# rishihahs/pupperv3-mjx

Measured on AMD Instinct MI355X. Metric: env-steps/sec at N_envs=4096/GPU, 1/2/4/8 MI355X; qpos rel-err vs mj_step, higher is better.
Workload: dtype f32

## Files before the change

### pupperv3-mjx_amd/csrc/pp3_device.h

```cpp
#pragma once
#include <hip/hip_runtime.h>
#include <stdint.h>

#include "pupper_hip.h"

namespace pp3 {

constexpr int NB = PP3_NBODY;
constexpr int NJ = PP3_NJNT;
constexpr int NV = PP3_NV;
constexpr int NQ = PP3_NQ;
constexpr int NU = PP3_NU;
constexpr int WAVE = 64;
constexpr int NLMAX = 12;
constexpr int NFR = 12;
constexpr int MAX_ROBOT_GEOM = 16;
constexpr int NMPAIR_MAX = 128;
constexpr int NMPAIR = 117;
constexpr int PAIR_REC = 24;

enum { PK_PLANE_SPHERE = 0, PK_SPHERE_SPHERE = 1, PK_SPHERE_BOX = 2 };
struct alignas(16) PairRec {
  int32_t kind, s1, s2;
  float r1, r2, margin;
  float p1[3], p2[3];
  float R[9];
  float half[3];
};
static_assert(sizeof(PairRec) == PAIR_REC * 4, "PairRec layout");
struct alignas(16) TerrainRec {
  float p[3];
  float R[9];
  float half[3];
  float pad;
};
static_assert(sizeof(TerrainRec) == 64, "TerrainRec layout");
struct alignas(16) PairCon {
  int32_t sup;
  uint32_t dm[2];
  float mu;
  float tran;
  float margin, b, k;
  float solimp[5];
  float knee, body;
  float pad;
};
static_assert(sizeof(PairCon) == 64, "PairCon layout");
static_assert(offsetof(PairCon, knee) == 52, "PairCon: knee/body in the 4th 16-byte word group");

template <int N>
struct alignas(16) LaneRec {
  float f[4 * N];
};
template <int N>
struct alignas(16) LaneTab {
  float g[N][32][4];
};
struct alignas(16) PairTab {
  float g[PAIR_REC / 4][PP3_MAX_PAIR][4];
};
enum {
  LL_LIM_ON = 0, LL_RANGE, LL_MARGIN, LL_INVW, LL_B, LL_K, LL_SOLIMP,
  LL_FR_R = 11, LL_FR_B, LL_ACT_DOF, LL_ACT_QADR, LL_ACT_FLAGS, LL_CRANGE,
  LL_GEAR = 18, LL_GAIN, LL_BIAS,
  LL_FRANGE = 23,
  LL_WORDS = 25
};
enum { ACTF_CTRLLIMITED = 1, ACTF_FORCELIMITED = 2, ACTF_AFFINE = 4 };
enum { LC_IQUAT = 0, LC_PT_BODY = 4, LC_PT_POS = 5, LC_WORDS = 8 };
enum { LM_IJ = 0, LM_ARM = 4, LM_DAMP = 8, LM_FLOSS = 9, LM_WORDS = 10 };
enum { LE_POSE = 0, LE_JLO, LE_JHI, LE_ABD, LE_LEG, LE_POSE16, LE_WORDS = 6 };
enum { LS_TYPE = 0, LS_ADR, LS_CUT, LS_BODY, LS_SPOS, LS_SQUAT = 7, LS_NCH = 11, LS_CH = 12, LS_MAXCH = 4,
       LS_WORDS = LS_CH + 4 * LS_MAXCH };

constexpr float MINVAL = 1e-15f;
constexpr float MINIMP = 0.0001f;
constexpr float MAXIMP = 0.9999f;

struct DevModel {
  LaneTab<(LL_WORDS + 3) / 4> lane_lim;
  LaneTab<(LC_WORDS + 3) / 4> lane_com;
  LaneTab<(LM_WORDS + 3) / 4> lane_m;
  float h;
  float gravity[3];
  float impratio;
  float gtol_scale;
  int32_t ls_iterations;
  int32_t iterations;
  float body_pos[NB][3];
  float body_quat[NB][4];
  float body_iquat[NB][4];
  float body_ipos[NB][3];
  float body_mass[NB];
// ... 283 lines not shown
```

### pupperv3-mjx_amd/csrc/pp3_env.hip

```cpp
#include <hip/hip_runtime.h>

#include <float.h>
#include <math.h>
#include <stddef.h>
#include <stdio.h>
#include <stdlib.h>
#include <string.h>

#include <string>
#include <algorithm>
#include <vector>

#include "pp3_device.h"
#include "pp3_diag.h"
#include "pp3_mlp.h"

namespace pp3 {

constexpr int HW = 32;
typedef __attribute__((address_space(4))) const DevModel GModel;
typedef __attribute__((address_space(4))) const float GFloat;
constexpr int HMAX = 16;
constexpr int OBS_MOVE = (PP3_OBS_DIM * (HMAX - 1) + HW - 1) / HW;
constexpr int NROBOT_GEOM = 8;
// ... 53 lines not shown
  float con_G[NC][5];
  float Jc[NC][3][NV];
  int lim_dof[NLMAX];
  float lim_sgn[NLMAX];
  float efc_D[NEFC], efc_R[NEFC], efc_aref[NEFC], efc_force[NEFC];
  Scratch<NC> x;
};

#define SYNC() asm volatile("" ::: "memory")
typedef float v4f __attribute__((ext_vector_type(4)));
#define PIN(...) asm volatile("" : __VA_ARGS__)
template <int N, int STRIDE>
__device__ __forceinline__ LaneRec<N> fetch_groups(const float* p) {
  v4f v[N];
#pragma unroll
  for (int k = 0; k < N; k++) v[k] = *reinterpret_cast<const v4f*>(p + k * STRIDE);
  if constexpr (N == 1) PIN("+v"(v[0]));
  else if constexpr (N == 2) PIN("+v"(v[0]), "+v"(v[1]));
  else if constexpr (N == 3) PIN("+v"(v[0]), "+v"(v[1]), "+v"(v[2]));
  else if constexpr (N == 4) PIN("+v"(v[0]), "+v"(v[1]), "+v"(v[2]), "+v"(v[3]));
  else if constexpr (N == 7) PIN("+v"(v[0]), "+v"(v[1]), "+v"(v[2]), "+v"(v[3]), "+v"(v[4]), "+v"(v[5]), "+v"(v[6]));
  else static_assert(N == 1, "fetch_rec: add a PIN arity");
  LaneRec<N> r;
#pragma unroll
  for (int k = 0; k < N; k++)
#pragma unroll
    for (int c = 0; c < 4; c++) r.f[4 * k + c] = v[k][c];
  return r;
}
template <int N>
__device__ __forceinline__ LaneRec<N> fetch_rec(const LaneRec<N>& src) {
  return fetch_groups<N, 4>(src.f);
}
template <int N>
__device__ __forceinline__ LaneRec<N> fetch_rec(const LaneTab<N>& t, int l) {
  return fetch_groups<N, 4 * 32>(t.g[0][l]);
}
__device__ __forceinline__ int as_i(float f) { return __float_as_int(f); }

__device__ __forceinline__ float frcp(float x) { return __builtin_amdgcn_rcpf(x); }
__device__ __forceinline__ float dpp_shr4(float v) {
  return __int_as_float(__builtin_amdgcn_update_dpp(0, __float_as_int(v), 0x114, 0xF, 0xF, true));
}

constexpr int HEAVY_WEIGHT = 5;

__device__ __forceinline__ float hb(float v, int k, int h) {
  const float a = rlane(v, k), b = rlane(v, k + HW);
  return h ? b : a;
}
__device__ __forceinline__ uint32_t hbu(uint32_t v, int k, int h) {
  const uint32_t a = (uint32_t)__builtin_amdgcn_readlane((int)v, k);
  const uint32_t b = (uint32_t)__builtin_amdgcn_readlane((int)v, k + HW);
  return h ? b : a;
}
__device__ __forceinline__ Key hkey(Key k, int l, int h) { return Key{hbu(k.a, l, h), hbu(k.b, l, h)}; }
__device__ __forceinline__ float hsum(float v, int) {
  v += dpp_f<0xB1, 0xF>(v, 0.0f);
  v += dpp_f<0x4E, 0xF>(v, 0.0f);
  v += dpp_f<0x141, 0xF>(v, 0.0f);
  v += dpp_f<0x140, 0xF>(v, 0.0f);
  const auto r = __builtin_amdgcn_permlane16_swap(__float_as_uint(v), __float_as_uint(v), false, false);
  return __uint_as_float(r[0]) + __uint_as_float(r[1]);
}
__device__ __forceinline__ float hsum_lane16(float v) {
  v += dpp_f<0xB1, 0xF>(v, 0.0f);
  v += dpp_f<0x4E, 0xF>(v, 0.0f);
  v += dpp_f<0x141, 0xF>(v, 0.0f);
  v += dpp_f<0x140, 0xF>(v, 0.0f);
// ... 250 lines not shown
    float t[10];
#pragma unroll
    for (int k = 0; k < 10; k++) t[k] = hsum_lane16(ci[k]);
    if (l == 16)
#pragma unroll
      for (int k = 0; k < 10; k++) s.crb_base[k] = t[k];
  }
  if (geom || foot) {
    float* dst = geom ? s.gxpos[l] : s.foot_xpos[l - 16];
    for (int k = 0; k < 3; k++) dst[k] = gpos[k];
  }
}

__device__ __forceinline__ void make_frame(float f[9], const float nin[3]) {
  float a[3] = {nin[0], nin[1], nin[2]};
  float n = sqrtf(dot3(a, a));
  if (n < MINVAL) { a[0] = 1; a[1] = 0; a[2] = 0; } else { const float in = 1.0f / n; a[0] *= in; a[1] *= in; a[2] *= in; }
  float y[3] = {0, 0, 0};
  if (a[1] < 0.5f && a[1] > -0.5f) y[1] = 1; else y[2] = 1;
  float ad = dot3(a, y);
  for (int k = 0; k < 3; k++) y[k] -= a[k] * ad;
  float yn = sqrtf(dot3(y, y));
  if (yn < MINVAL) { y[0] = 1; y[1] = 0; y[2] = 0; } else { const float in = 1.0f / yn; y[0] *= in; y[1] *= in; y[2] *= in; }
  float z[3];
  cross3(z, a, y);
  for (int k = 0; k < 3; k++) { f[k] = a[k]; f[3 + k] = y[k]; f[6 + k] = z[k]; }
}

struct PairLoad {
  v4f v[7];
};
__device__ __forceinline__ PairLoad load_pair(const DevModel& m, int p) {
  PairLoad r;
#pragma unroll
  for (int k = 0; k < 6; k++) r.v[k] = *reinterpret_cast<const v4f*>(m.pair_rec.g[k][p]);
  r.v[6] = *reinterpret_cast<const v4f*>(&m.pair_con[p]);
  return r;
}
struct TerrainRef {
  uint64_t terrain;
  int nbox;
};
template <int NC, int NWV = 1>
__device__ __forceinline__ bool narrow(const Shared<NC>& s, const TerrainRef& tr, PairLoad pl, float& dist, float pos[3],
                                       float nrm[3], v4f& pc0) {
  PairRec rec;
  {
    PIN("+v"(pl.v[0]), "+v"(pl.v[1]), "+v"(pl.v[2]), "+v"(pl.v[3]), "+v"(pl.v[4]), "+v"(pl.v[5]), "+v"(pl.v[6]));
    __builtin_memcpy(&rec, pl.v, sizeof(rec));
    pc0 = pl.v[6];
  }
  const float margin = rec.margin;
  float p1[3], p2[3];
  {
    const int i1 = rec.s1 >= 0 ? rec.s1 : 0, i2 = rec.s2 >= 0 ? rec.s2 : 0;
    float l1[3], l2[3];
#pragma unroll
    for (int k = 0; k < 3; k++) { l1[k] = s.gxpos[i1][k]; l2[k] = s.gxpos[i2][k]; }
    asm volatile("" : "+v"(l1[0]), "+v"(l1[1]), "+v"(l1[2]), "+v"(l2[0]), "+v"(l2[1]), "+v"(l2[2]));
#pragma unroll
    for (int k = 0; k < 3; k++) {
      p1[k] = rec.s1 >= 0 ? l1[k] : rec.p1[k];
      p2[k] = rec.s2 >= 0 ? l2[k] : rec.p2[k];
    }
  }
  if (rec.kind == PK_PLANE_SPHERE) {
    const float nz[3] = {rec.R[2], rec.R[5], rec.R[8]};
    const float v[3] = {p2[0] - p1[0], p2[1] - p1[1], p2[2] - p1[2]};
    const float r = rec.r2;
// ... 367 lines not shown
  for (int k = 0; k < NV - 1; ++k) {
    const float yk = hb(x, k, h);
    x = (l > k) ? x - a[k] * yk : x;
  }
  x = x * dinv;
  SYNC();
  float col[NV];
#pragma unroll
  for (int k = 1; k < NV; ++k) col[k] = s.x.L[k][li];
#pragma unroll
  for (int k = NV - 1; k > 0; --k) {
    const float xk = hb(x, k, h);
    x = (l < k) ? x - col[k] * xk : x;
  }
  return x;
}

__host__ __device__ constexpr int pnat(int p) { return p < 12 ? p + 6 : p - 12; }
__host__ __device__ constexpr int npos(int d) { return d < 6 ? d + 12 : d - 6; }

__device__ __forceinline__ float dpp_shl1(float v) { return dpp_f<0x101, 0xF>(v, 0.0f); }
__device__ __forceinline__ float dpp_shl2(float v) { return dpp_f<0x102, 0xF>(v, 0.0f); }

__device__ __forceinline__ float ldl_arrow_solve(float (&a)[NV], float b, int l, float* col ) {
  l = opaque_lane(l);
  const int slot = l < NV ? l : NV;
  const int lp = l < NV ? l : NV - 1;
  const int pg = lp < 12 ? lp / 3 : 0, pst = lp < 12 ? lp - 3 * pg : 3;
  float mydiag = 1.0f;
#pragma unroll
  for (int st = 0; st < 3; st++) {
#pragma unroll
    for (int g = 0; g < 4; g++) col[20 * g + slot] = a[3 * g + st];
    if (l < 12 && l - 3 * (l / 3) == st) col[20 * (l / 3) + 19] = b;
    SYNC();
    {
      const float pv = col[20 * pg + slot];
      mydiag = (pst == st) ? pv : mydiag;
    }
#pragma unroll
    for (int g = 0; g < 4; g++) {
      const int k = 3 * g + st;
      const float* c = col + 20 * g;
      float r[20];
#pragma unroll
      for (int qq = 0; qq < 2; qq++) {
        const int q = ((3 * g) & ~3) + 4 * qq;
        if (q < 12 && q <= 3 * g + 2) {
          const float4 v = *reinterpret_cast<const float4*>(c + q);
          r[q] = v.x; r[q + 1] = v.y; r[q + 2] = v.z; r[q + 3] = v.w;
        }
      }
#pragma unroll
      for (int q = 12; q < 20; q += 4) {
        const float4 v = *reinterpret_cast<const float4*>(c + q);
        r[q] = v.x; r[q + 1] = v.y; r[q + 2] = v.z; r[q + 3] = v.w;
      }
      float ik = frcp(fmaxf(r[k], MINVAL));
      PIN("+v"(ik));
      const float lik = (l > k) ? a[k] * ik : 0.0f;
#pragma unroll
      for (int jj = 0; jj < 3; ++jj)
        if (jj > st) a[3 * g + jj] -= lik * r[3 * g + jj];
#pragma unroll
      for (int j = 12; j < NV; ++j) a[j] -= lik * r[j];
      b -= lik * r[19];
    }
    SYNC();
  }
  if (l >= 12 && l < NV) {
#pragma unroll
    for (int c = 0; c < 6; c++) col[6 * (l - 12) + c] = a[12 + c];
    col[36 + (l - 12)] = b;
  }
  SYNC();
  float S[6][6], y[6];
#pragma unroll
  for (int q = 0; q < 36; q += 4) {
    const float4 v = *reinterpret_cast<const float4*>(col + q);
    S[q / 6][q % 6] = v.x; S[(q + 1) / 6][(q + 1) % 6] = v.y;
    S[(q + 2) / 6][(q + 2) % 6] = v.z; S[(q + 3) / 6][(q + 3) % 6] = v.w;
  }
  {
    const float4 v0 = *reinterpret_cast<const float4*>(col + 36);
    const float2 v1 = *reinterpret_cast<const float2*>(col + 40);
    y[0] = v0.x; y[1] = v0.y; y[2] = v0.z; y[3] = v0.w; y[4] = v1.x; y[5] = v1.y;
  }
  SYNC();
  float db[6];
#pragma unroll
  for (int k = 0; k < 6; ++k) {
    const float ik = frcp(fmaxf(S[k][k], MINVAL));
    db[k] = ik;
#pragma unroll
    for (int i = 5; i > k; --i) {
      const float lik = S[i][k] * ik;
#pragma unroll
      for (int j = k + 1; j <= i; ++j) S[i][j] -= lik * S[j][k];
      S[i][k] = lik;
    }
  }
#pragma unroll
  for (int c = 1; c < 6; c++)
#pragma unroll
    for (int k = 0; k < c; k++) y[c] = y[c] - S[c][k] * y[k];
#pragma unroll
// ... 333 lines not shown
  }
  const int li = l < NV ? l : NV - 1;
  float a[NV], dinv = 1.0f;
#pragma unroll
  for (int j = 0; j < NV; j++) a[j] = s.M[li][j];
  const float dD = s.dofD[li];
#pragma unroll
  for (int j = 0; j < NV; j++) a[j] += (j == li) ? dD : 0.0f;
  for (int c = 0; c < cmax; c++) {
    if (c < ncon) {
      const float* G = s.con_G[c];
      const float jn = s.Jc[c][0][li], j1 = s.Jc[c][1][li], j2 = s.Jc[c][2][li];
      const float w0 = jn * G[0] + j1 * G[1] + j2 * G[2];
      const float w1 = jn * G[1] + j1 * G[3];
      const float w2 = jn * G[2] + j2 * G[4];
      hess_acc<0, NV>(a, s.Jc[c], w0, w1, w2);
    }
  }
  ldl_rows(a, dinv, l, &s.x.L[0][0]);
  const float x = ldl_solve(s, a, dinv, s.grad[li], l, h);
  if (l < NV) s.search[l] = -x;
}

template <int NC, int NWV = 1, bool LIBSC = true, bool CULL = false>
__device__ __forceinline__ int substep(Shared<NC>& s, const DevModel& m, int l, int h, bool integrate_prev,
                                       const KinConst& kc PROF_PARAM, float* ccache = nullptr) {
  constexpr int NR = (Shared<NC>::NEFC + HW - 1) / HW;
  l = opaque_lane(l);
  LaneRec<2> rc_pf;
  LaneRec<3> rm_pf;
  {
    v4f v[5];
#pragma unroll
    for (int k = 0; k < 2; k++) v[k] = *reinterpret_cast<const v4f*>(m.lane_com.g[k][l]);
#pragma unroll
    for (int k = 0; k < 2; k++)
      for (int c = 0; c < 4; c++) rc_pf.f[4 * k + c] = v[k][c];
#pragma unroll
    for (int k = 0; k < 3; k++) v[2 + k] = *reinterpret_cast<const v4f*>(m.lane_m.g[k][l]);
#pragma unroll
    for (int k = 0; k < 3; k++)
      for (int c = 0; c < 4; c++) rm_pf.f[4 * k + c] = v[2 + k][c];
  }
  kinematics<NC, LIBSC>(s, m, l, integrate_prev, kc); SYNC();
  PHASE(0); l = opaque_lane(l);
  { com_pos(s, m, l, h, rc_pf); SYNC(); }
  PHASE(1); l = opaque_lane(l);
  const PairLoad pair_pf = load_pair(m, l < m.npair ? l : 0);
  { crb_times_cdof(s, m, l); rne_chain(s, m, l); SYNC(); }
  PHASE(15); l = opaque_lane(l);
  int lsup = 4;
  { lsup = collision<NC, NWV, CULL>(s, m, l, h, pair_pf, ccache); SYNC(); }
  PHASE(16); l = opaque_lane(l);
  v4f pcv[4];
  {
    const int c = l >> 2;
    const int p = c < s.ncon ? s.con_pair[c < NC ? c : 0] : 0;
    const v4f* src = reinterpret_cast<const v4f*>(&m.pair_con[p]);
#pragma unroll
    for (int k = 0; k < 4; k++) pcv[k] = src[k];
  }
  {
    const LaneRec<7> rl = fetch_rec(m.lane_lim, l);
    const int jlim = l < 2 * (NJ - 1) ? 1 + (l >> 1) : 1;
    const bool actl = l < NU;
    const int adof = actl ? as_i(rl.f[LL_ACT_DOF]) : 0, aqadr = actl ? as_i(rl.f[LL_ACT_QADR]) : 0;
    float lq = s.qpos[7 + jlim - 1], lqv = s.qvel[6 + jlim - 1], fqv = s.qvel[6 + (l < NFR ? l : 0)];
    float actrl = s.ctrl[actl ? l : 0], aq = s.qpos[aqadr], aqv = s.qvel[adof];
    float skp = s.kp, skd = s.kd;
    int sdr = s.dr_on;
    PIN("+v"(lq), "+v"(lqv), "+v"(fqv), "+v"(actrl), "+v"(aq), "+v"(aqv), "+v"(skp), "+v"(skd), "+v"(sdr));
    bool act = false;
    float value = 0;
    int j = 0;
    if (l < 2 * (NJ - 1)) {
      j = 1 + (l >> 1);
      const float side = (l & 1) ? 1.0f : -1.0f;
      if (as_i(rl.f[LL_LIM_ON])) {
        value = side * (rl.f[LL_RANGE] - lq);
        act = value < rl.f[LL_MARGIN];
      }
    }
    const uint32_t mask = hballot(act, h);
    const int slot = __popc(mask & ((1u << l) - 1u));
    if (act && slot < NLMAX) {
      const int dof = 6 + j - 1;
      const float sg = (l & 1) ? -1.0f : 1.0f;
      s.lim_dof[slot] = dof;
      s.lim_sgn[slot] = sg;
      const float imp = getimp(&rl.f[LL_SOLIMP], value, rl.f[LL_MARGIN]);
      const float R = fmaxf(MINVAL, (1.0f - imp) / imp * rl.f[LL_INVW]);
// ... 122 lines not shown
  const int nefc = NFR + nl + 4 * ncon;
  for (int e = l; e < 4 * ncon; e += HW) {
    const int c = e >> 2, p = s.con_pair[c], r = NFR + nl + e;
    LaneRec<4> pc;
    if (e < HW) {
#pragma unroll
      for (int k = 0; k < 4; k++)
#pragma unroll
        for (int cc = 0; cc < 4; cc++) pc.f[4 * k + cc] = pcv[k][cc];
    } else {
      pc = fetch_rec(*reinterpret_cast<const LaneRec<4>*>(&m.pair_con[p]));
    }
    const PairCon& q = *reinterpret_cast<const PairCon*>(&pc);
    const float mu = s.con_mu[c];
    const float dist = s.con_dist[c];
    const float vel = row_dot(s, r, nl, ncon, s.qvel);
    const float tran = q.tran;
    const float invw = (tran + mu * mu * tran) * 2.0f * mu * mu / m.impratio;
    const float imp = getimp(q.solimp, dist, q.margin);
    const float R = fmaxf(MINVAL, (1.0f - imp) / imp * invw);
    s.efc_R[r] = R;
    s.efc_D[r] = 1.0f / R;
    s.efc_aref[r] = -q.b * vel - q.k * imp * (dist - q.margin);
  }
  SYNC();
  PHASE(13); l = opaque_lane(l);
  float mrow[NV];
  {
    const int lp = l < NV ? l : NV - 1, dn = pnat(lp);
    float a[NV];
#pragma unroll
    for (int j = 0; j < NV; j++) { a[j] = s.M[dn][pnat(j)]; mrow[j] = a[j]; }
    const float x = ldl_arrow_solve(a, s.qfrc_smooth[dn], l, &s.x.L[0][0]);
    if (l < NV) s.qacc_smooth[dn] = x;
  }
  SYNC();
  PHASE(4); l = opaque_lane(l);

  float Dr[NR], Rr[NR], ar[NR], fl[NR];
  bool valid[NR], isfr[NR];
#pragma unroll
  for (int t = 0; t < NR; t++) {
    const int r = l + HW * t;
    valid[t] = r < nefc;
    isfr[t] = r < NFR;
    Dr[t] = valid[t] ? s.efc_D[r] : 0.0f;
    Rr[t] = valid[t] ? s.efc_R[r] : 0.0f;
    ar[t] = valid[t] ? s.efc_aref[r] : 0.0f;
    fl[t] = (valid[t] && isfr[t]) ? rm.f[LM_FLOSS] : 0.0f;
  }
  float cws = 0, csm = 0;
  float xws[NR], xsm[NR], ma_ws = 0.0f;
  bool use_smooth;
  {
#pragma unroll
    for (int t = 0; t < NR; t++) {
      xws[t] = 0.0f;
      xsm[t] = 0.0f;
      if (!valid[t]) continue;
      const int r = l + HW * t;
      float d1, d2;
      row_dot2(s, r, nl, ncon, s.qws, s.qacc_smooth, d1, d2);
      const float x1 = d1 - ar[t];
      const float x2 = d2 - ar[t];
      xws[t] = x1;
      xsm[t] = x2;
      const float rf = Rr[t] * fl[t];
      const float q1 = 0.5f * Dr[t] * x1 * x1, q2 = 0.5f * Dr[t] * x2 * x2;
      const float f1 = (x1 <= -rf) ? (-fl[t] * x1 - 0.5f * rf * fl[t]) : (x1 >= rf) ? (fl[t] * x1 - 0.5f * rf * fl[t]) : q1;
      const float f2 = (x2 <= -rf) ? (-fl[t] * x2 - 0.5f * rf * fl[t]) : (x2 >= rf) ? (fl[t] * x2 - 0.5f * rf * fl[t]) : q2;
      cws += isfr[t] ? f1 : ((x1 < 0) ? q1 : 0.0f);
      csm += isfr[t] ? f2 : ((x2 < 0) ? q2 : 0.0f);
    }
    PHASE(23);
    if (l < NV) {
      const int dn = pnat(l);
      ma_ws = mrow_dot_reg(mrow, s.qws);
      cws += 0.5f * (ma_ws - s.qfrc_smooth[dn]) * (s.qws[dn] - s.qacc_smooth[dn]);
    }
    cws = hsum(cws, h);
    csm = hsum(csm, h);
    use_smooth = cws > csm;
    if (l < NV) s.qacc[l] = use_smooth ? s.qacc_smooth[l] : s.qws[l];
  }
  SYNC();
  PHASE(5); l = opaque_lane(l);
  const int cmax = wmax2(ncon);
  __builtin_assume(cmax >= 0 && cmax <= NC);
  int weight = cmax;
  bool live = true;
  for (int iter = 0; iter < m.iterations; iter++) {
    float ma = 0;
    if (l < NV) {
      if (iter > 0 || use_smooth) ma = mrow_dot_reg(mrow, s.qacc);
      else ma = ma_ws;
    }
    float jar[NR];
#pragma unroll
    for (int t = 0; t < NR; t++) {
      jar[t] = 0;
      if (!valid[t]) continue;
      const int r = l + HW * t;
      const float x = iter > 0 ? row_dot(s, r, nl, ncon, s.qacc) - ar[t] : (use_smooth ? xsm[t] : xws[t]);
      jar[t] = x;
      const float rf = Rr[t] * fl[t];
      const float fq = -Dr[t] * x;
      const bool lo = isfr[t] && x <= -rf;
      const bool hi = !lo && (isfr[t] ? x >= rf : x >= 0);
      const float f = lo ? fl[t] : (hi ? (isfr[t] ? -fl[t] : 0.0f) : fq);
      const float Dq = (lo || hi) ? 0.0f : Dr[t];
      s.efc_force[r] = f;
      s.efc_D[r] = Dq;
    }
    SYNC();
    PHASE(22);
    float gauss = 0;
// ... 45 lines not shown
        const float dD = s.dofD[dn];
        const uint32_t onehot = 1u << lp;
#pragma unroll
        for (int j = 0; j < NV; j++) a[j] = fmaf(dD, (float)((onehot >> j) & 1u), a[j]);
        for (int c = 0; c < cmax; c++) {
          const bool cv = c < ncon;
          const int sa = __builtin_amdgcn_readlane(lsup, c), sb = __builtin_amdgcn_readlane(lsup, HW + c);
          const uint32_t legs = (1u << (sa & 7)) | (1u << (sb & 7));
          if (cv) {
            float G[5], jb[3][6];
#pragma unroll
            for (int k = 0; k < 5; k++) G[k] = s.con_G[c][k];
            float jn = s.Jc[c][0][dn], j1 = s.Jc[c][1][dn], j2 = s.Jc[c][2][dn];
#pragma unroll
            for (int r = 0; r < 3; r++)
#pragma unroll
              for (int j = 0; j < 6; j++) jb[r][j] = s.Jc[c][r][j];
            PIN("+v"(G[0]), "+v"(G[1]), "+v"(G[2]), "+v"(G[3]), "+v"(G[4]), "+v"(jn), "+v"(j1), "+v"(j2),
                "+v"(jb[0][0]), "+v"(jb[0][1]), "+v"(jb[0][2]), "+v"(jb[0][3]), "+v"(jb[0][4]), "+v"(jb[0][5]),
                "+v"(jb[1][0]), "+v"(jb[1][1]), "+v"(jb[1][2]), "+v"(jb[1][3]), "+v"(jb[1][4]), "+v"(jb[1][5]),
                "+v"(jb[2][0]), "+v"(jb[2][1]), "+v"(jb[2][2]), "+v"(jb[2][3]), "+v"(jb[2][4]), "+v"(jb[2][5]));
            const float w0 = jn * G[0] + j1 * G[1] + j2 * G[2];
            const float w1 = jn * G[1] + j1 * G[3];
            const float w2 = jn * G[2] + j2 * G[4];
            hess_acc_p<0, 6>(a, jb, w0, w1, w2);
            if (legs & 1u) hess_acc_p<6, 9>(a, s.Jc[c], w0, w1, w2);
            if (legs & 2u) hess_acc_p<9, 12>(a, s.Jc[c], w0, w1, w2);
            if (legs & 4u) hess_acc_p<12, 15>(a, s.Jc[c], w0, w1, w2);
            if (legs & 8u) hess_acc_p<15, 18>(a, s.Jc[c], w0, w1, w2);
          }
        }
        PHASE(14); l = opaque_lane(l);
        const float x = ldl_arrow_solve(a, s.grad[dn], l, &s.x.L[0][0]);
        if (l < NV) s.search[dn] = -x;
      } else {
        dense_search<NC>((LdsShared<NC>*)&s, l, h, cmax, ncon, lsup);
      }
    }
    SYNC();
    PHASE(7); l = opaque_lane(l);
    float q1 = 0, q2 = 0, sn = 0;
    if (l < NV) {
      const int dn = pnat(l);
      const float sv = s.search[dn];
      const float mv = mrow_dot_reg(mrow, s.search);
      q1 = sv * (ma - s.qfrc_smooth[dn]);
      q2 = 0.5f * sv * mv;
      sn = sv * sv;
    }
    float jv[NR];
#pragma unroll
    for (int t = 0; t < NR; t++) jv[t] = valid[t] ? row_dot(s, l + HW * t, nl, ncon, s.search) : 0.0f;
    float thr_lo[NR], thr_hi[NR], cq[NR][3], clo[NR][2], chi[NR][2];
    bool rowany[NR];
#pragma unroll
    for (int t = 0; t < NR; t++) {
      const float D = Dr[t], jr = jar[t], jw = jv[t];
      cq[t][0] = valid[t] ? 0.5f * D * jr * jr : 0.0f;
      cq[t][1] = valid[t] ? D * jr * jw : 0.0f;
      cq[t][2] = valid[t] ? 0.5f * D * jw * jw : 0.0f;
      const float rf = Rr[t] * fl[t];
      const bool fr = valid[t] && isfr[t];
      thr_lo[t] = fr ? -rf : -INFINITY;
      thr_hi[t] = fr ? rf : (valid[t] ? 0.0f : INFINITY);
      clo[t][0] = fr ? -fl[t] * jr - 0.5f * rf * fl[t] : 0.0f;
      clo[t][1] = fr ? -fl[t] * jw : 0.0f;
      chi[t][0] = fr ? fl[t] * jr - 0.5f * rf * fl[t] : 0.0f;
// ... 97 lines not shown
  if (g2 * (CG) > 0 && fabsf(CG) < fabsf(g2)) { a2 = CA; c2 = CC; g2 = CG; h2 = CH; up2 = true; }
            PP3_TIGHTEN(a1n, c1n, g1n, h1n)
            PP3_TIGHTEN(a2n, c2n, g2n, h2n)
            PP3_TIGHTEN(am, cm, gm, hm)
#undef PP3_TIGHTEN
            if (!up1 && !up2) break;
            if (up1) { a1n = a1 - g1 / h1; eval(a1n, c1n, g1n, h1n); evals++; }
            if (up2) { a2n = a2 - g2 / h2; eval(a2n, c2n, g2n, h2n); evals++; }
          }
          if (!finished) alpha = c1 < c2 ? a1 : a2;
        }
      }
    }
#ifdef PP3_PHASE_PROF
    {
      const int ew = wmax2(evals);
      if (pf) pf->evals += ew;
      PROF_ADD(19, ew);
      PROF_ADD(20, evals);
      PROF_ADD(HW + 20, evals);
    }
#endif
    PHASE(8); l = opaque_lane(l);
#ifdef PP3_DEBUG
    if (blockIdx.x == 0 && h == 0) {
      if (l < NV) { g_dbg[l] = s.qacc[l]; g_dbg[18 + l] = s.grad[l]; g_dbg[36 + l] = s.search[l]; }
      if (l == 0) {
        g_dbg[54] = gauss; g_dbg[55] = q1; g_dbg[56] = q2; g_dbg[57] = sn; g_dbg[58] = gtol;
        g_dbg[59] = alpha; g_dbg[60] = (float)evals; g_dbg[61] = cws; g_dbg[62] = csm; g_dbg[63] = (float)nefc;
      }
    }
#endif
    live = live && alpha != 0.0f;
    if (live && l < NV) s.qacc[l] += alpha * s.search[l];
    SYNC();
  }
  if (l < NV) s.qws[l] = s.qacc[l];
  if (l < NV) s.efc_aref[l] = s.qvel[l];
  SYNC();
  return weight;
}

template <int NC, bool LIBSC = true>
__device__ __forceinline__ void euler_step(Shared<NC>& s, const DevModel& m, int l) {
  const float hstep = m.h;
  float vn = 0;
  float w[3] = {0, 0, 0};
  if (l < NV) vn = s.qvel[l] + hstep * s.qacc[l];
  if (l == 3)
    for (int k = 0; k < 3; k++) w[k] = s.qvel[3 + k] + hstep * s.qacc[3 + k];
  SYNC();
  if (l < NV) s.qvel[l] = vn;
  if (l < 3) s.qpos[l] += hstep * vn;
  if (l >= 6 && l < NV) s.qpos[l + 1] += hstep * vn;
  if (l == 3) {
    const float n = sqrtf(dot3(w, w));
    if (n < MINVAL) { w[0] = 1; w[1] = 0; w[2] = 0; } else { const float in = 1.0f / n; w[0] *= in; w[1] *= in; w[2] *= in; }
    float qr[4], q[4] = {s.qpos[3], s.qpos[4], s.qpos[5], s.qpos[6]};
    axisangle2quat<LIBSC>(qr, w, hstep * n);
    normalize4(q);
    mulquat(q, q, qr);
    for (int k = 0; k < 4; k++) s.qpos[3 + k] = q[k];
  }
  SYNC();
}

template <int NC>
__device__ __forceinline__ void load_params(Shared<NC>& s, const DevModel& m, const float* dr, int l) {
  if (l < NB) {
    s.mass[l] = dr ? dr[PP3_DR_MASS + l] : m.body_mass[l];
    for (int k = 0; k < 3; k++) {
// ... 615 lines not shown
  float fa = s.qfrc_act[l18], fa6 = s.qfrc_act[6 + l12], qv = s.qvel[6 + l12], qp = s.qpos[7 + l12];
  float lvel = s.st[PP3_S_LAST_VEL + l12], lact = s.st[PP3_S_LAST_ACT + l12];
  float airt = s.st[PP3_S_AIR_TIME + l4], fst = s.x.e.first[l4];
  float sp[3], xb[3], xdab[3], xdvb[2];
#pragma unroll
  for (int k = 0; k < 3; k++) { sp[k] = s.foot_xpos[l4][k]; xb[k] = s.xpos[bleg][k]; xdab[k] = s.x.e.xda[bleg][k]; }
  xdvb[0] = s.x.e.xdv[bleg][0];
  xdvb[1] = s.x.e.xdv[bleg][1];
  int fcm = s.x.e.filt_cm[l4], ncon_r = s.ncon, cpair = s.con_pair[lc];
  float cdist = s.con_dist[lc];
  PIN("+v"(fa), "+v"(fa6), "+v"(qv), "+v"(qp), "+v"(lvel), "+v"(lact), "+v"(airt), "+v"(fst), "+v"(sp[0]), "+v"(sp[1]),
      "+v"(sp[2]), "+v"(xb[0]), "+v"(xb[1]), "+v"(xb[2]), "+v"(xdab[0]), "+v"(xdab[1]), "+v"(xdab[2]), "+v"(xdvb[0]),
      "+v"(xdvb[1]), "+v"(fcm), "+v"(ncon_r), "+v"(cpair), "+v"(cdist));
  if (l < NV) r_torq = fa * fa;
  if (l < 12) {
    const float acc = (qv - lvel) / m.env_dt;
    r_jacc = acc * acc;
    r_mech = fabsf(fa6 * qv);
    const float da = act_in - lact;
    r_arate = da * da;
    r_stand = fabsf(qp - re.f[LE_POSE]);
    r_standv = fabsf(qv);
    if (l % 3 == 1) { const float t = qp - re.f[LE_ABD]; r_abd = t * t; }
  }
  if (l < 4) {
    r_air = (airt - 0.1f) * fst;
    const float off[3] = {sp[0] - xb[0], sp[1] - xb[1], sp[2] - xb[2]};
    float cr[3];
    cross3(cr, xdab, off);
    const float vx = xdvb[0] + cr[0], vy = xdvb[1] + cr[1];
    r_slip = (vx * vx + vy * vy) * (fcm ? 1.0f : 0.0f);
  }
  if (l < ncon_r && cdist < 0.0f) {
    const v4f kb = reinterpret_cast<const v4f*>(&m.pair_con[cpair])[3];
    r_knee = kb[1];
    r_body = kb[2];
  }
  r_torq = hsum(r_torq, h);
  r_jacc = hsum(r_jacc, h);
  r_mech = hsum(r_mech, h);
  r_arate = hsum(r_arate, h);
  r_stand = hsum(r_stand, h) * ((cn < 0.1f) ? 1.0f : 0.0f);
  r_standv = hsum(r_standv, h) * ((cn < m.stand_thr) ? 1.0f : 0.0f);
  r_abd = hsum(r_abd, h);
  r_air = hsum(r_air, h) * ((cn > 0.05f) ? 1.0f : 0.0f);
  r_slip = hsum(r_slip, h);
  r_knee = hsum(r_knee, h);
  r_body = hsum(r_body, h);
  float rw[PP3_NREWARD];
  {
    const float inv[4] = {s.xquat[1][0], -s.xquat[1][1], -s.xquat[1][2], -s.xquat[1][3]};
    const float sig = m.sigma;
    const float* xdv1 = s.x.e.xdv[1];
    const float* xda1 = s.x.e.xda[1];
    float lv[3], av[3], wz[3], ru[3];
    b_rotate(lv, xdv1, inv);
    b_rotate(av, xda1, inv);
    b_rotate(wz, z0, inv);
    b_rotate(ru, z0, s.xquat[1]);
    const float e_lin = (cmd0 - lv[0]) * (cmd0 - lv[0]) + (cmd1 - lv[1]) * (cmd1 - lv[1]);
    float e_ori = 0;
    for (int k = 0; k < 3; k++) e_ori += (wz[k] - s.st[PP3_S_DESIRED_Z + k]) * (wz[k] - s.st[PP3_S_DESIRED_Z + k]);
    rw[PP3_REWARD_TRACKING_LIN_VEL] = expf(-e_lin / sig);
    rw[PP3_REWARD_TRACKING_ANG_VEL] = expf(-(cmd2 - av[2]) * (cmd2 - av[2]) / sig);
    rw[PP3_REWARD_TRACKING_ORIENTATION] = expf(-e_ori / sig);
    rw[PP3_REWARD_LIN_VEL_Z] = xdv1[2] * xdv1[2];
    rw[PP3_REWARD_ANG_VEL_XY] = xda1[0] * xda1[0] + xda1[1] * xda1[1];
// ... 602 lines not shown
    d->pair_tran[p] = (float)(mm->body_invweight0[mm->cgeom_bodyid[g1]][0] + mm->body_invweight0[mm->cgeom_bodyid[g2]][0]);
    {
      auto cls = [](int b) { return b == 0 ? -1 : (b == 1 ? 4 : (b - 2) / 3); };
      const int c1 = cls(mm->cgeom_bodyid[g1]), c2 = cls(mm->cgeom_bodyid[g2]);
      int sup;
      if (c1 < 0) sup = c2;
      else if (c2 < 0) sup = c1;
      else if (c1 == c2) sup = c1;
      else if (c1 == 4) sup = c2;
      else if (c2 == 4) sup = c1;
      else sup = 5 | 8 | ((c1 < c2 ? c1 : c2) << 4) | ((c1 < c2 ? c2 : c1) << 6);
      d->pair_sup[p] = sup < 0 ? 5 : sup;
    }
    d->pair_dm[p][0] = d->body_dofmask[mm->cgeom_bodyid[g1]];
    d->pair_dm[p][1] = d->body_dofmask[mm->cgeom_bodyid[g2]];
    {
      PairRec r;
      memset(&r, 0, sizeof(r));
      const int t1 = mm->cgeom_type[g1], t2 = mm->cgeom_type[g2];
      r.kind = (t1 == PP3_GEOM_PLANE && t2 == PP3_GEOM_SPHERE) ? PK_PLANE_SPHERE
               : (t1 == PP3_GEOM_SPHERE && t2 == PP3_GEOM_SPHERE) ? PK_SPHERE_SPHERE
               : (t1 == PP3_GEOM_SPHERE && t2 == PP3_GEOM_BOX) ? PK_SPHERE_BOX : -1;
      r.s1 = d->cg_slot[g1];
      r.s2 = r.kind == PK_SPHERE_BOX ? -1 - box_slot[g2] : d->cg_slot[g2];
      r.r1 = d->cg_size[g1][0];
      r.r2 = d->cg_size[g2][0];
      r.margin = d->pair_margin[p];
      for (int k = 0; k < 3; k++) { r.p1[k] = d->cg_pos[g1][k]; r.p2[k] = d->cg_pos[g2][k]; }
      const int gf = r.kind == PK_SPHERE_BOX ? g2 : g1;
      for (int k = 0; k < 9; k++) r.R[k] = d->cg_wmat[gf][k];
      if (r.kind == PK_SPHERE_BOX)
        for (int k = 0; k < 3; k++) r.half[k] = d->cg_size[g2][k];
      const float* rf = reinterpret_cast<const float*>(&r);
      for (int k = 0; k < PAIR_REC / 4; k++)
        for (int c = 0; c < 4; c++) d->pair_rec.g[k][p][c] = rf[4 * k + c];
    }
    {
      PairCon& q = d->pair_con[p];
      memset(&q, 0, sizeof(q));
      q.sup = d->pair_sup[p];
      q.dm[0] = d->pair_dm[p][0];
      q.dm[1] = d->pair_dm[p][1];
      q.mu = d->pair_mu[p];
      q.tran = d->pair_tran[p];
      q.margin = d->pair_margin[p];
      q.b = d->pair_b[p];
      q.k = d->pair_k[p];
      for (int k = 0; k < 5; k++) q.solimp[k] = d->pair_solimp[p][k];
    }
    if (mm->cgeom_margin[g1] != 0 || mm->cgeom_margin[g2] != 0) return set_err(PP3_ERR_MODEL, "nonzero geom margins unsupported");
  }
  {
    d->cull_on = 0;
    d->cull_reach = 0.0f;
    memset(d->pair_box4, 0xFF, sizeof(d->pair_box4));
    memset(d->box_tab, 0, sizeof(d->box_tab));
    bool ok = d->nbox >= 1 && d->nbox <= 32 && d->npair > 32 && d->npair <= 32 * 5 && mm->body_parentid[1] == 0;
    const char* off = getenv("PP3_NO_CULL");
    if (off && off[0] == '1') ok = false;
    double reach = 0.0, margin = 0.0;
    for (int sl = 0; ok && sl < d->nrobot_geom; sl++) {
      const int g = d->robot_geom[sl];
      const double* gp = mm->cgeom_pos[g];
      double dist = sqrt(gp[0] * gp[0] + gp[1] * gp[1] + gp[2] * gp[2]);
      int b = mm->cgeom_bodyid[g];
      for (; b > 1; b = mm->body_parentid[b]) {
        const double* bp = mm->body_pos[b];
        dist += sqrt(bp[0] * bp[0] + bp[1] * bp[1] + bp[2] * bp[2]);
      }
      if (b != 1) ok = false;
      reach = fmax(reach, dist + mm->cgeom_size[g][0]);
    }
    for (int p = 0; ok && p < d->npair; p++) {
      const int g1 = mm->pair_g1[p], g2 = mm->pair_g2[p];
      const bool sb = mm->cgeom_type[g1] == PP3_GEOM_SPHERE && mm->cgeom_type[g2] == PP3_GEOM_BOX && box_slot[g2] >= 0;
      if (sb) margin = fmax(margin, (double)d->pair_margin[p]);
      if (p >= 32 && sb) {
        const int k = p / 32 - 1, ln = p % 32;
        d->pair_box4[ln] = (d->pair_box4[ln] & ~(0xFFu << (8 * k))) | ((uint32_t)box_slot[g2] << (8 * k));
      }
    }
// ... 751 lines not shown
```

Measured before the change: 51.93 million.

## Tile pair table into 32-pair batches with inlined first PairCon group

```diff
diff --git a/pupperv3-mjx_amd/csrc/pp3_device.h b/pupperv3-mjx_amd/csrc/pp3_device.h
--- a/pupperv3-mjx_amd/csrc/pp3_device.h
+++ b/pupperv3-mjx_amd/csrc/pp3_device.h
@@ -56,9 +56,14 @@
 struct alignas(16) LaneTab {
   float g[N][32][4];
 };
+constexpr int PAIR_GROUPS = PAIR_REC / 4 + 1;
 struct alignas(16) PairTab {
-  float g[PAIR_REC / 4][PP3_MAX_PAIR][4];
-};
+  float g[PP3_MAX_PAIR / 32][PAIR_GROUPS][32][4];
+};
+static_assert(PP3_MAX_PAIR % 32 == 0, "PairTab: whole 32-pair batches");
+__host__ __device__ constexpr unsigned pair_tab_byte(unsigned p) {
+  return (p >> 5) * (unsigned)(PAIR_GROUPS * 512) + (p & 31u) * 16u;
+}
 enum {
   LL_LIM_ON = 0, LL_RANGE, LL_MARGIN, LL_INVW, LL_B, LL_K, LL_SOLIMP,
   LL_FR_R = 11, LL_FR_B, LL_ACT_DOF, LL_ACT_QADR, LL_ACT_FLAGS, LL_CRANGE,
diff --git a/pupperv3-mjx_amd/csrc/pp3_env.hip b/pupperv3-mjx_amd/csrc/pp3_env.hip
--- a/pupperv3-mjx_amd/csrc/pp3_env.hip
+++ b/pupperv3-mjx_amd/csrc/pp3_env.hip
@@ -109,9 +109,23 @@
 __device__ __forceinline__ LaneRec<N> fetch_rec(const LaneRec<N>& src) {
   return fetch_groups<N, 4>(src.f);
 }
+template <class T>
+__device__ __forceinline__ const float* at_bytes(const T& tab, unsigned off) {
+  return reinterpret_cast<const float*>(reinterpret_cast<const char*>(&tab) + off);
+}
+typedef __attribute__((address_space(1))) const v4f GV4;
+template <class T>
+__device__ __forceinline__ const GV4* far_groups(const T& tab, unsigned off) {
+  uint64_t b = (uint64_t)(uintptr_t)&tab;
+  asm("" : "+s"(b));
+  return (const GV4*)(uintptr_t)(b + off);
+}
 template <int N>
 __device__ __forceinline__ LaneRec<N> fetch_rec(const LaneTab<N>& t, int l) {
-  return fetch_groups<N, 4 * 32>(t.g[0][l]);
+  return fetch_groups<N, 4 * 32>(at_bytes(t, 16u * (unsigned)l));
+}
+__device__ __forceinline__ const GV4* pair_con_groups(const DevModel& m, int p) {
+  return far_groups(m.pair_con, (unsigned)sizeof(PairCon) * (unsigned)p);
 }
 __device__ __forceinline__ int as_i(float f) { return __float_as_int(f); }
 
@@ -428,9 +442,9 @@
 };
 __device__ __forceinline__ PairLoad load_pair(const DevModel& m, int p) {
   PairLoad r;
-#pragma unroll
-  for (int k = 0; k < 6; k++) r.v[k] = *reinterpret_cast<const v4f*>(m.pair_rec.g[k][p]);
-  r.v[6] = *reinterpret_cast<const v4f*>(&m.pair_con[p]);
+  const GV4* g = far_groups(m.pair_rec, pair_tab_byte((unsigned)p));
+#pragma unroll
+  for (int k = 0; k < PAIR_GROUPS; k++) r.v[k] = g[32 * k];
   return r;
 }
 struct TerrainRef {
@@ -864,7 +878,7 @@
   for (int st = 0; st < 3; st++) {
 #pragma unroll
     for (int g = 0; g < 4; g++) col[20 * g + slot] = a[3 * g + st];
-    if (l < 12 && l - 3 * (l / 3) == st) col[20 * (l / 3) + 19] = b;
+    col[(l < 12 && pst == st) ? 20 * pg + 19 : NV] = b;
     SYNC();
     {
       const float pv = col[20 * pg + slot];
@@ -900,10 +914,12 @@
     }
     SYNC();
   }
-  if (l >= 12 && l < NV) {
-#pragma unroll
-    for (int c = 0; c < 6; c++) col[6 * (l - 12) + c] = a[12 + c];
-    col[36 + (l - 12)] = b;
+  {
+    const bool base_row = l >= 12 && l < NV;
+    const int so = base_row ? 6 * (l - 12) : 48, bo = base_row ? 36 + (l - 12) : 54;
+#pragma unroll
+    for (int c = 0; c < 6; c++) col[so + c] = a[12 + c];
+    col[bo] = b;
   }
   SYNC();
   float S[6][6], y[6];
@@ -1303,12 +1319,12 @@
   {
     v4f v[5];
 #pragma unroll
-    for (int k = 0; k < 2; k++) v[k] = *reinterpret_cast<const v4f*>(m.lane_com.g[k][l]);
+    for (int k = 0; k < 2; k++) v[k] = *reinterpret_cast<const v4f*>(at_bytes(m.lane_com, 16u * (unsigned)l) + k * 128);
 #pragma unroll
     for (int k = 0; k < 2; k++)
       for (int c = 0; c < 4; c++) rc_pf.f[4 * k + c] = v[k][c];
 #pragma unroll
-    for (int k = 0; k < 3; k++) v[2 + k] = *reinterpret_cast<const v4f*>(m.lane_m.g[k][l]);
+    for (int k = 0; k < 3; k++) v[2 + k] = *reinterpret_cast<const v4f*>(at_bytes(m.lane_m, 16u * (unsigned)l) + k * 128);
 #pragma unroll
     for (int k = 0; k < 3; k++)
       for (int c = 0; c < 4; c++) rm_pf.f[4 * k + c] = v[2 + k][c];
@@ -1327,7 +1343,7 @@
   {
     const int c = l >> 2;
     const int p = c < s.ncon ? s.con_pair[c < NC ? c : 0] : 0;
-    const v4f* src = reinterpret_cast<const v4f*>(&m.pair_con[p]);
+    const GV4* src = pair_con_groups(m, p);
 #pragma unroll
     for (int k = 0; k < 4; k++) pcv[k] = src[k];
   }
@@ -1516,7 +1532,7 @@
 #pragma unroll
     for (int j = 0; j < NV; j++) { a[j] = s.M[dn][pnat(j)]; mrow[j] = a[j]; }
     const float x = ldl_arrow_solve(a, s.qfrc_smooth[dn], l, &s.x.L[0][0]);
-    if (l < NV) s.qacc_smooth[dn] = x;
+    s.qacc_smooth[dn] = x;
   }
   SYNC();
   PHASE(4); l = opaque_lane(l);
@@ -1565,7 +1581,10 @@
     cws = hsum(cws, h);
     csm = hsum(csm, h);
     use_smooth = cws > csm;
-    if (l < NV) s.qacc[l] = use_smooth ? s.qacc_smooth[l] : s.qws[l];
+    {
+      const int lc = l < NV ? l : NV - 1;
+      s.qacc[lc] = use_smooth ? s.qacc_smooth[lc] : s.qws[lc];
+    }
   }
   SYNC();
   PHASE(5); l = opaque_lane(l);
@@ -1677,7 +1696,7 @@
         }
         PHASE(14); l = opaque_lane(l);
         const float x = ldl_arrow_solve(a, s.grad[dn], l, &s.x.L[0][0]);
-        if (l < NV) s.search[dn] = -x;
+        s.search[dn] = -x;
       } else {
         dense_search<NC>((LdsShared<NC>*)&s, l, h, cmax, ncon, lsup);
       }
@@ -1841,11 +1860,19 @@
     }
 #endif
     live = live && alpha != 0.0f;
-    if (live && l < NV) s.qacc[l] += alpha * s.search[l];
+    {
+      const int lc = l < NV ? l : NV - 1;
+      const float qa = s.qacc[lc];
+      const float qn = qa + alpha * s.search[lc];
+      s.qacc[lc] = live ? qn : qa;
+    }
     SYNC();
   }
-  if (l < NV) s.qws[l] = s.qacc[l];
-  if (l < NV) s.efc_aref[l] = s.qvel[l];
+  {
+    const int lc = l < NV ? l : NV - 1;
+    s.qws[lc] = s.qacc[lc];
+    s.efc_aref[lc] = s.qvel[lc];
+  }
   SYNC();
   return weight;
 }
@@ -2527,7 +2554,7 @@
     r_slip = (vx * vx + vy * vy) * (fcm ? 1.0f : 0.0f);
   }
   if (l < ncon_r && cdist < 0.0f) {
-    const v4f kb = reinterpret_cast<const v4f*>(&m.pair_con[cpair])[3];
+    const v4f kb = pair_con_groups(m, cpair)[3];
     r_knee = kb[1];
     r_body = kb[2];
   }
@@ -3196,8 +3223,9 @@
       if (r.kind == PK_SPHERE_BOX)
         for (int k = 0; k < 3; k++) r.half[k] = d->cg_size[g2][k];
       const float* rf = reinterpret_cast<const float*>(&r);
+      float* g = reinterpret_cast<float*>(reinterpret_cast<char*>(&d->pair_rec) + pair_tab_byte((unsigned)p));
       for (int k = 0; k < PAIR_REC / 4; k++)
-        for (int c = 0; c < 4; c++) d->pair_rec.g[k][p][c] = rf[4 * k + c];
+        for (int c = 0; c < 4; c++) g[128 * k + c] = rf[4 * k + c];
     }
     {
       PairCon& q = d->pair_con[p];
@@ -3211,6 +3239,7 @@
       q.b = d->pair_b[p];
       q.k = d->pair_k[p];
       for (int k = 0; k < 5; k++) q.solimp[k] = d->pair_solimp[p][k];
+      memcpy(reinterpret_cast<char*>(&d->pair_rec) + pair_tab_byte((unsigned)p) + 512 * (PAIR_GROUPS - 1), &q, 16);
     }
     if (mm->cgeom_margin[g1] != 0 || mm->cgeom_margin[g2] != 0) return set_err(PP3_ERR_MODEL, "nonzero geom margins unsupported");
   }
```

After: 52.59 million (median of 6 runs). 1.01x the previous value.
